# keychera/raytracing-clj

Hardware: AMD Instinct MI355X
Metric: Mray-samples/sec at 1200×675×100spp depth50; achieved HBM GB/s vs peak (higher is better)
Workload: dtype fp32

## Files before the change

raytracing-clj_amd/csrc/bvh.cpp:

```cpp
#include "bvh.h"

#include <algorithm>
#include <climits>
#include <cmath>
#include <numeric>

namespace rtclj {

float g_bvh_big_ratio = 4.0f;

namespace {

struct Box {
  float lo[3] = {INFINITY, INFINITY, INFINITY};
  float hi[3] = {-INFINITY, -INFINITY, -INFINITY};
  void add(const Box& b) {
    for (int k = 0; k < 3; ++k) {
      lo[k] = std::min(lo[k], b.lo[k]);
      hi[k] = std::max(hi[k], b.hi[k]);
    }
  }
};

Box body_box(const float* s) {
// ... 142 lines not shown
    std::nth_element(tmp.begin(), tmp.begin() + n / 2, tmp.end());
    med = tmp[n / 2];
  }
  Builder b{sph, {}, out};
  b.leaf_size = leaf_size;
  b.sah = sah;
  std::vector<char> is_big(n, 0);
  for (int i = 0; i < n; ++i) {
    const bool finite = std::isfinite(sph[4 * i]) && std::isfinite(sph[4 * i + 1]) &&
                        std::isfinite(sph[4 * i + 2]) && std::isfinite(sph[4 * i + 3]);
    if (!finite && out->big.size() < 64) {
      is_big[i] = 1;
      out->big.push_back(i);
    }
  }
  if (n > 8) {
    std::vector<int> order(n);
    std::iota(order.begin(), order.end(), 0);
    std::stable_sort(order.begin(), order.end(), [&](int x, int y) { return radii[x] > radii[y]; });
    int added = 0;
    for (int i : order) {
      if (added == kBvhBigMax || !(radii[i] > g_bvh_big_ratio * med)) break;
      if (is_big[i]) continue;
      is_big[i] = 1;
      out->big.push_back(i);
      ++added;
    }
  }
  std::sort(out->big.begin(), out->big.end());
  for (int i = 0; i < n; ++i)
    if (!is_big[i]) b.prim.push_back(i);
  Box all;
  for (int i : b.prim) all.add(body_box(sph + 4 * i));
  double bc[3] = {0, 0, 0}, br = 0;
  if (!b.prim.empty()) {
    for (int k = 0; k < 3; ++k) bc[k] = 0.5 * (double(all.lo[k]) + all.hi[k]);
    for (int i : b.prim) {
      const float* s = sph + 4 * i;
      const double dx = s[0] - bc[0], dy = s[1] - bc[1], dz = s[2] - bc[2];
      br = std::max(br, std::sqrt(dx * dx + dy * dy + dz * dz) + std::fabs(s[3]));
    }
  }
  for (int k = 0; k < 3; ++k) out->center[k] = static_cast<float>(bc[k]);
  out->radius = static_cast<float>(br * (1.0 + 1e-6)) + 1e-6f;
  out->nodes.emplace_back();
  const int cnt = static_cast<int>(b.prim.size());
  Box b0, b1;
  int c0 = 0, c1 = 0;
  if (cnt == 0) {
    c0 = c1 = b.leaf(0, 0, &b0);
    for (int k = 0; k < 3; ++k) b0.lo[k] = b0.hi[k] = 0.0f;
    b1 = b0;
  } else if (cnt <= leaf_size) {
    c0 = c1 = b.leaf(0, cnt, &b0);
    b1 = b0;
  } else {
    const int mid = b.split(0, cnt, 0);
    c0 = b.build(0, mid, 1, &b0);
    c1 = b.build(mid, cnt, 1, &b1);
  }
  BvhNode& root = out->nodes[0];
  set_box(root, 0, b0);
  set_box(root, 1, b1);
  root.child[0] = c0;
  root.child[1] = c1;
  for (BvhNode& nd : out->nodes) {
    float* ax[3] = {nd.x, nd.y, nd.z};
    for (int k = 0; k < 3; ++k)
      for (int c = 0; c < 2; ++c) {
        ax[k][c] = std::nextafter(static_cast<float>(double(ax[k][c]) - out->center[k]), -INFINITY);
        ax[k][2 + c] = std::nextafter(static_cast<float>(double(ax[k][2 + c]) - out->center[k]), INFINITY);
        ax[k][4 + c] = ax[k][c];
      }
  }
  out->depth = b.max_depth + 1;
  out->big_pair0 = static_cast<int>(out->pidx.size() / 2);
  const int nb = static_cast<int>(out->big.size());
// ... 11 lines not shown
```

raytracing-clj_amd/csrc/bvh.h:

```cpp
#pragma once
#include <cstdint>
#include <vector>

namespace rtclj {

struct alignas(16) BvhNode {
  float x[6], y[6], z[6];
  int child[2];
};
static_assert(sizeof(BvhNode) == 80, "BvhNode layout");

struct BvhHost {
  std::vector<BvhNode> nodes;
  std::vector<float> pairs;
  std::vector<int> pidx;
  std::vector<int> big;
  int big_pair0 = 0;
  int n_big_leaves = 0;
  float center[3] = {0, 0, 0};
  float radius = 0.0f;
  int depth = 0;
  int leaf_size = 2;
};

constexpr int kBvhStack = 16;
constexpr int kBvhBigMax = 8;

int bvh_build(const float* sphere, int n, BvhHost* out, int leaf_size = 2, bool sah = true);

}
```

raytracing-clj_amd/csrc/trace.hip:

```cpp
#include "trace_kernel.h"

#include <algorithm>
#include <chrono>
#include <atomic>
#include <climits>
#include <cstdlib>
#include <cmath>
#include <cstdint>
#include <cstring>
#include <mutex>
#include <string>
#include <thread>
#include <type_traits>
#include <vector>

namespace rtclj {

__device__ __forceinline__ int cost_bucket(unsigned c) {
  if (c < 8) return static_cast<int>(c);
  const int e = 31 - __clz(c);
  return ((e - 2) << 3) | static_cast<int>((c >> (e - 3)) & 7u);
}
__global__ __launch_bounds__(1024) void order_kernel(unsigned* __restrict__ cost, int* __restrict__ order,
                                                     int n) {
// ... 176 lines not shown
    case 28: return v28;
  }
#ifdef RTCLJ_DIAG
  if (const Variant* d = diag_variant(v)) return *d;
#endif
  return none;
}
static std::atomic<int> g_variant{0};
static std::atomic<int> g_schedule{0};
static const bool g_bvh_sah = [] {
  const char* e = std::getenv("RTCLJ_BVH");
  return !(e && std::strcmp(e, "median") == 0);
}();
#ifdef RTCLJ_DIAG
static const bool g_timeline = [] {
  const char* e = std::getenv("RTCLJ_TIMELINE");
  return e && std::atoi(e) != 0;
}();
#endif
constexpr int kDbg = 32;
constexpr int kDbgDevices = 64;
static std::mutex g_dbg_mu;
static unsigned long long* g_dbg[kDbgDevices] = {};
static unsigned long long* g_dbgw[kDbgDevices] = {};

}

using namespace rtclj;

struct DTree {
  float4* blob;
  int blob_f4, off_pairs, off_pidx, big_pair0, n_big_leaves, depth, n_nodes;
  float c[3], r;
};

struct ScheduleKey {
  int width, rows, row_begin, row_tile, tile_first, tile_step, gx, gy;
};
struct Schedule {
  hipStream_t stream = nullptr;
  unsigned* cost = nullptr;
  int* order = nullptr;
  int cap = 0;
  bool ready = false;
  bool sort_pending = false;
  int sort_plan = -1;
  ScheduleKey key{};
  unsigned long long* part = nullptr;
  size_t part_cap = 0;
  bool part_dirty = false;
  unsigned long long* word = nullptr;
  unsigned* done = nullptr;
  unsigned long long* sum = nullptr;
  int steal_cap = 0;
  int* owner = nullptr;
  int owner_cap = 0;
  unsigned long long* stealc = nullptr;
  unsigned epoch = 0;
  bool epoch_started = false;
  int2* units = nullptr;
  int units_cap = 0;
  int plan_units = -1;
  uint4* xq = nullptr;
  size_t xq_cap = 0;
  unsigned* xq_n = nullptr;
  unsigned long long xq_launches = 0;
// ... 171 lines not shown
    std::thread th[2];
    for (int k = 1; k < 3; ++k) th[k - 1] = std::thread([&, k] { bvh_build(s->sphere, n, &bvhs[k], 2 << k, g_bvh_sah); });
    bvh_build(s->sphere, n, &bvhs[0], 2, g_bvh_sah);
    for (std::thread& t : th) t.join();
  }
  hipError_t e = hipMalloc(&d->geo, n_pad * sizeof(float4));
  for (int k = 0; k < 3 && e == hipSuccess; ++k) {
    BvhHost& bvh = bvhs[k];
    const size_t nb = bvh.nodes.size() * sizeof(BvhNode);
    const size_t pb = bvh.pairs.size() * sizeof(float);
    const size_t isz = k == 2 ? sizeof(uint16_t) : sizeof(int);
    std::vector<uint16_t> pidx16(bvh.pidx.size());
    for (size_t i = 0; i < pidx16.size(); ++i) pidx16[i] = static_cast<uint16_t>(bvh.pidx[i]);
    const size_t ib = ((bvh.pidx.size() * isz + 15) / 16) * 16;
    std::vector<char> blob(nb + pb + ib, 0);
    if (k == 1)
      for (BvhNode& nd : bvh.nodes)
        for (int& c : nd.child)
          if (c >= 0) c *= static_cast<int>(sizeof(BvhNode));
    std::memcpy(blob.data(), bvh.nodes.data(), nb);
    std::memcpy(blob.data() + nb, bvh.pairs.data(), pb);
    if (k == 2) std::memcpy(blob.data() + nb + pb, pidx16.data(), pidx16.size() * sizeof(uint16_t));
    else std::memcpy(blob.data() + nb + pb, bvh.pidx.data(), bvh.pidx.size() * sizeof(int));
    DTree& t = d->tree[k];
    t.blob_f4 = static_cast<int>(blob.size() / 16);
    t.off_pairs = static_cast<int>(nb);
    t.off_pidx = static_cast<int>(nb + pb);
    t.big_pair0 = bvh.big_pair0;
    t.n_big_leaves = bvh.n_big_leaves;
    t.depth = bvh.depth;
    t.n_nodes = static_cast<int>(bvh.nodes.size());
    for (int j = 0; j < 3; ++j) t.c[j] = bvh.center[j];
    t.r = bvh.radius;
    e = hipMalloc(&t.blob, blob.size());
    if (e == hipSuccess) e = hipMemcpy(t.blob, blob.data(), blob.size(), hipMemcpyHostToDevice);
  }
  if (e == hipSuccess) e = hipMalloc(&d->geo2, n_pad * sizeof(float4));
  if (e == hipSuccess) e = hipMemcpy(d->geo2, geo2.data(), n_pad * sizeof(float4), hipMemcpyHostToDevice);
  if (e == hipSuccess) e = hipMalloc(&d->sph, cnt * sizeof(float4));
  if (e == hipSuccess) e = hipMalloc(&d->mat, cnt * sizeof(float4));
  if (e == hipSuccess) e = hipMalloc(&d->kind, cnt * sizeof(int));
  if (e == hipSuccess) e = hipMemcpy(d->geo, geo.data(), n_pad * sizeof(float4), hipMemcpyHostToDevice);
  if (e == hipSuccess) e = hipMemcpy(d->sph, sph.data(), cnt * sizeof(float4), hipMemcpyHostToDevice);
  if (e == hipSuccess) e = hipMemcpy(d->mat, mat.data(), cnt * sizeof(float4), hipMemcpyHostToDevice);
  if (e == hipSuccess) e = hipMemcpy(d->kind, kind.data(), cnt * sizeof(int), hipMemcpyHostToDevice);
  if (e != hipSuccess) {
    rt_scene_free(d);
    return hip_fail(e, "rt_scene_upload");
  }
  {
    std::lock_guard<std::mutex> lk(g_scenes_mu);
    g_scenes.push_back(d);
  }
  *out = d;
  return RT_OK;
}

extern "C" int rt_scene_free(rt_dscene* d) {
  if (!d) return RT_OK;
  {
    std::lock_guard<std::mutex> lk(g_scenes_mu);
    g_scenes.erase(std::remove(g_scenes.begin(), g_scenes.end(), d), g_scenes.end());
  }
  (void)hipSetDevice(d->device);
  if (d->geo) (void)hipFree(d->geo);
  if (d->geo2) (void)hipFree(d->geo2);
// ... 225 lines not shown
  std::memcpy(a.cam + 12, c->disk_u, 12);
  std::memcpy(a.cam + 15, c->disk_v, 12);
  a.defocus = c->defocus ? 1 : 0;
  a.n = ds->n;
  a.n_pad = ds->n_pad;
  a.width = p->width;
  a.rows_out = rows;
  a.row_begin = p->row_begin;
  a.row_tile = p->row_tile > 0 ? p->row_tile : 8;
  a.tile_first = p->tile_first;
  a.tile_step = p->tile_step;
  a.spp = p->spp;
  a.sample_begin = p->sample_begin;
  a.max_depth = p->max_depth;
  a.realm = (p->flags & RT_FLAG_REALM) ? 1 : 0;
  a.sampler = (p->flags & RT_FLAG_REJECTION_SAMPLERS) ? 0 : (RT_SAMPLER_SPHERE | RT_SAMPLER_DISK);
  a.key = seed_key(p->seed);
  if (rows == 0) return RT_OK;
  HIP_TRY(hipSetDevice(ds->device));
  int vsel = launch_variant(*ds, *p);
  if (variant_table(vsel).scan == SCAN_BVHS && p->max_depth > 1023) vsel = 16;
  const Variant& v = variant_table(vsel);
  if (!v.fn) return set_error(RT_E_ARG, "rt_launch: no kernel for variant " + std::to_string(vsel));
  const DTree& tr = ds->tree[variant_tree(vsel)];
  a.bvh_blob = tr.blob;
  a.bvh_blob_f4 = tr.blob_f4;
  a.bvh_off_pairs = tr.off_pairs;
  a.bvh_off_pidx = tr.off_pidx;
  a.big_pair0 = tr.big_pair0;
  a.n_big_leaves = tr.n_big_leaves;
  a.bvh_stack = compact_variant(vsel) ? stack_entries_compact(tr) : stack_entries(tr, variant_tree(vsel));
  for (int k = 0; k < 3; ++k) a.bvh_c[k] = tr.c[k];
  a.bvh_r = tr.r;
  {
    const int words = a.bvh_stack * 16 * (v.scan == SCAN_BVHO || v.scan == SCAN_BVHQ7 ? 1 : 2);
    a.mb_paths = std::min(32, words / kMbFields);
    a.compact = is_bvh_scan(v.scan) ? std::min(a.mb_paths, env_int("RTCLJ_COMPACT", a.mb_paths, 0)) : 0;
  }
  hipStream_t stream = static_cast<hipStream_t>(hip_stream);
  const int th = variant_rows(v);
  const int gx = (p->width + kTile - 1) / kTile, gy = (rows + th - 1) / th;
  const dim3 block(v.threads);
  const int n_tiles = gx * gy;
  a.tiles_x = gx;
  if (v.stats) {
    const int rc = dbg_buffers(ds->device, &a.dbg, &a.dbgw);
    if (rc != RT_OK) return rc;
  }
#ifdef RTCLJ_DIAG
  else if (g_timeline) {
    unsigned long long* unused = nullptr;
    const int rc = dbg_buffers(ds->device, &unused, &a.dbgw);
    if (rc != RT_OK) return rc;
  }
#endif
#ifdef RTCLJ_DIAG
  const size_t lds = launch_lds(*ds, vsel) + static_cast<size_t>(env_int("RTCLJ_LDS_PAD", 0, 0));
#else
  const size_t lds = launch_lds(*ds, vsel);
#endif
  if (lds > 64 * 1024) {
    HIP_TRY(hipFuncSetAttribute(v.fn, hipFuncAttributeMaxDynamicSharedMemorySize, static_cast<int>(lds)));
    if (v.sweep) HIP_TRY(hipFuncSetAttribute(v.sweep, hipFuncAttributeMaxDynamicSharedMemorySize, static_cast<int>(lds)));
  }
  Schedule* sch = nullptr;
  std::unique_lock<std::mutex> sched_lock;
// ... 344 lines not shown
```

raytracing-clj_amd/csrc/trace_diag.hip:

```cpp
#include "trace_kernel.h"

namespace rtclj {

template <int SRC, int SCAN, class F>
__device__ void diag_scan(const KArgs& a, const float4* s_geo, float ox, float oy, float oz, float ux, float uy,
                          float uz, F&& consider) {
  const int n = a.n;
  if constexpr (SCAN == SCAN_SIMPLE) {
#pragma unroll 1
    for (int s = 0; s < n; ++s) {
      float4 g;
      if constexpr (SRC == SRC_LDS) g = s_geo[s];
      else g = a.geo[s];
      const float ocx = g.x - ox, ocy = g.y - oy, ocz = g.z - oz;
      const float h = fmaf(uz, ocz, fmaf(uy, ocy, ux * ocx));
      const float c = fmaf(ocx, ocx, fmaf(ocz, ocz, fmaf(ocy, ocy, g.w)));
      const float disc = fmaf(h, h, -c);
      if ((disc >= 0.0f) & ((h >= 0.0f) | (c < 0.0f))) consider(h, disc, s);
    }
  } else {
    const Pair* tab;
    if constexpr (SRC == SRC_LDS) tab = reinterpret_cast<const Pair*>(s_geo);
    else tab = a.geo2;
    const f2 ox2 = {ox, ox}, oy2 = {oy, oy}, oz2 = {oz, oz};
// ... 231 lines not shown
        ox = cx;
        oy = cy;
        oz = cz;
      }
      dx = sx - ox;
      dy = sy - oy;
      dz = sz - oz;
      tr = tg = tb = 1.0f;
      rem = a.max_depth;
      last = -1;
      j = -1;
    }
    bool done = false;
    --rem;
    ++segs;
    const float len = sqrt_rn(fmaf(dz, dz, fmaf(dy, dy, dx * dx)));
    const float il = 1.0f / len;
    const float ux = dx * il, uy = dy * il, uz = dz * il;
    const float tmin = 1e-3f * len;
    float best_t = INFINITY;
    int best = -1;
    {
      auto consider_tie = [&](float h, float disc, int s) {
        const float sq = (s == last) ? fabsf(h) : sqrt_rn(disc);
        const float tn = h - sq;
        const float t = tn > tmin ? tn : h + sq;
        const uint64_t kk = (static_cast<uint64_t>(__float_as_uint(t)) << 32) | static_cast<uint32_t>(s);
        const uint64_t bkey = (static_cast<uint64_t>(__float_as_uint(best_t)) << 32) | static_cast<uint32_t>(best);
        const bool acc = (t > tmin) & (kk < bkey);
        best_t = acc ? t : best_t;
        best = acc ? s : best;
      };
      const float ecx = ox - a.bvh_c[0], ecy = oy - a.bvh_c[1], ecz = oz - a.bvh_c[2];
      const float D = __builtin_amdgcn_sqrtf(fmaf(ecz, ecz, fmaf(ecy, ecy, ecx * ecx))) + a.bvh_r;
      const float P = fmaf(2e-3f, D, 1e-6f);
      const float rux = __builtin_amdgcn_fmed3f(__builtin_amdgcn_rcpf(ux), -1e24f, 1e24f);
      const float ruy = __builtin_amdgcn_fmed3f(__builtin_amdgcn_rcpf(uy), -1e24f, 1e24f);
      const float ruz = __builtin_amdgcn_fmed3f(__builtin_amdgcn_rcpf(uz), -1e24f, 1e24f);
      f2 r_xy = {rux, ruy}, r_z = {ruz, ruz};
      const float nlx = -(ecx + P) * rux, nly = -(ecy + P) * ruy, nlz = -(ecz + P) * ruz;
      const float nhx = -(ecx - P) * rux, nhy = -(ecy - P) * ruy, nhz = -(ecz - P) * ruz;
      const bool sx = rux < 0.0f, sy = ruy < 0.0f, sz = ruz < 0.0f;
      f2 nf_x = {sx ? nhx : nlx, sx ? nlx : nhx};
      f2 nf_y = {sy ? nhy : nly, sy ? nly : nhy};
      f2 nf_z = {sz ? nhz : nlz, sz ? nlz : nhz};
      const int offx = sx ? 8 : 0, offy = 24 + (sy ? 8 : 0), offz = 48 + (sz ? 8 : 0);
      f2 o_xy = {ox, oy}, o_zux = {oz, ux}, u_yz = {uy, uz};
      auto leaf = [&](int p) {
        float hh[4], dd[4];
        int ii[4];
        unsigned nc[4];
        const Pair* const lp = pairs + p;
        const int2* const li = pidx + p;
#pragma unroll
        for (int qq = 0; qq < 2; ++qq) {
          const Pair g = lp[qq];
          const int2 id = li[qq];
          asm volatile("" : "+v"(o_xy), "+v"(o_zux), "+v"(u_yz));
          const f2 ocx = g.x - bc_lo(o_xy), ocy = g.y - bc_hi(o_xy), ocz = g.z - bc_lo(o_zux);
          const f2 h = fma2(bc_hi(u_yz), ocz, fma2(bc_lo(u_yz), ocy, bc_hi(o_zux) * ocx));
          const f2 c = fma2(ocx, ocx, fma2(ocz, ocz, fma2(ocy, ocy, g.w)));
          const f2 disc = fma2(h, h, -c);
          hh[2 * qq] = h.x;
          hh[2 * qq + 1] = h.y;
          dd[2 * qq] = disc.x;
          dd[2 * qq + 1] = disc.y;
          ii[2 * qq] = id.x;
          ii[2 * qq + 1] = id.y;
          const float d0 = disc.x, d1 = disc.y, h0 = h.x, h1 = h.y, c0 = c.x, c1 = c.y;
          nc[2 * qq] = __builtin_amdgcn_bitop3_b32(__float_as_uint(d0), __float_as_uint(h0), __float_as_uint(c0), 0x0b);
          nc[2 * qq + 1] = __builtin_amdgcn_bitop3_b32(__float_as_uint(d1), __float_as_uint(h1), __float_as_uint(c1), 0x0b);
        }
        const unsigned b01 = __builtin_amdgcn_perm(nc[1], nc[0], 0x0c0c0b09u);
        const unsigned b23 = __builtin_amdgcn_perm(nc[3], nc[2], 0x0b090c0cu);
        unsigned m = __builtin_amdgcn_bitop3_b32(b01, b23, 0x01010101u, 0xa8);
        while (m) {
          const unsigned k = __builtin_ctz(m);
          m &= m - 1;
          float h = hh[0], d = dd[0];
          int s = ii[0];
#pragma unroll
          for (int jj = 1; jj < 4; ++jj) {
            h = k == static_cast<unsigned>(8 * jj) ? hh[jj] : h;
            d = k == static_cast<unsigned>(8 * jj) ? dd[jj] : d;
            s = k == static_cast<unsigned>(8 * jj) ? ii[jj] : s;
          }
          consider_tie(h, d, s);
        }
      };
      auto node_test = [&](int node, float& tn0, float& tn1, bool& hit0, bool& hit1, int& c0, int& c1) {
        const char* nb = reinterpret_cast<const char*>(nodes) + static_cast<unsigned>(node);
        const f2* ax = reinterpret_cast<const f2*>(nb + offx);
        const f2* ay = reinterpret_cast<const f2*>(nb + offy);
        const f2* az = reinterpret_cast<const f2*>(nb + offz);
        const int2 ch = *reinterpret_cast<const int2*>(nb + 72);
        asm volatile("" : "+v"(r_xy), "+v"(r_z), "+v"(nf_x), "+v"(nf_y), "+v"(nf_z));
        const f2 tnx = fma2(ax[0], bc_lo(r_xy), bc_lo(nf_x)), tfx = fma2(ax[1], bc_lo(r_xy), bc_hi(nf_x));
        const f2 tny = fma2(ay[0], bc_hi(r_xy), bc_lo(nf_y)), tfy = fma2(ay[1], bc_hi(r_xy), bc_hi(nf_y));
        const f2 tnz = fma2(az[0], bc_lo(r_z), bc_lo(nf_z)), tfz = fma2(az[1], bc_lo(r_z), bc_hi(nf_z));
        tn0 = fmaxf(fmaxf(tnx.x, tny.x), tnz.x);
        tn1 = fmaxf(fmaxf(tnx.y, tny.y), tnz.y);
        const float tf0 = fminf(fminf(tfx.x, tfy.x), tfz.x);
        const float tf1 = fminf(fminf(tfx.y, tfy.y), tfz.y);
        float ntn0, ntn1;
        asm("v_max_f32 %0, %1, %2" : "=v"(ntn0) : "v"(tn0), "v"(tmin));
        asm("v_max_f32 %0, %1, %2" : "=v"(ntn1) : "v"(tn1), "v"(tmin));
        hit0 = ntn0 <= fminf(tf0, best_t);
        hit1 = ntn1 <= fminf(tf1, best_t);
        c0 = ch.x;
        c1 = ch.y;
      };
      for (int b = 0; b < a.n_big_leaves; ++b) leaf(a.big_pair0 + b * 2);
      int node = 0;
      unsigned short* top = stk0;
      bool go = true;
      while (go) {
        float tn0, tn1;
        bool hit0, hit1;
        int c0, c1;
        node_test(node, tn0, tn1, hit0, hit1, c0, c1);
        const bool l0 = hit0 && c0 < 0, l1 = hit1 && c1 < 0;
        if (l0 || l1) {
          leaf(l0 ? ~c0 : ~c1);
          if (l0 && l1) leaf(~c1);
        }
        const bool i0 = hit0 && !l0, i1 = hit1 && !l1;
        const bool sw = tn1 < tn0;
        int nxt = (i0 && (!i1 || !sw)) ? c0 : c1;
        *top = static_cast<unsigned short>(sw ? c0 : c1);
        top += (i0 && i1) ? 64 : 0;
        if (!(i0 || i1)) {
          go = top != stk0;
// ... 174 lines not shown
```

raytracing-clj_amd/csrc/trace_kernel.h:

```cpp
#pragma once
#include <hip/hip_runtime.h>

#include <algorithm>
#include <chrono>
#include <atomic>
#include <climits>
#include <cstdlib>
#include <cmath>
#include <cstdint>
#include <cstring>
#include <mutex>
#include <string>
#include <thread>
#include <type_traits>
#include <vector>

#include "bvh.h"
#include "fp_rn.h"
#include "rt_internal.h"

namespace rtclj {

struct alignas(16) KArgs {
  const float4* geo;
  const struct Pair* geo2;
  const float4* sph;
  const float4* mat;
  const int* kind;
  float* out;
  unsigned long long* counters;
  unsigned long long* dbg;
  unsigned long long* dbgw;
  float cam[18];
  int defocus;
  int n;
  int n_pad;
  int width;
  int rows_out;
  int row_begin, row_tile, tile_first, tile_step;
  const float4* bvh_blob;
  int bvh_blob_f4;
  int bvh_off_pairs;
  int bvh_off_pidx;
  int big_pair0;
  int n_big_leaves;
  int bvh_stack;
  float bvh_c[3], bvh_r;
  const int* tile_order;
  unsigned* tile_cost;
  unsigned long long* part;
  int tiles_x;
  int n_whole, split;
  const int2* unit_tab;
  uint64_t rt_magic;
  int spp, sample_begin, max_depth;
  int realm;
  int sampler;
  uint32_t key;
  unsigned long long* word;
  unsigned* done;
  unsigned long long* sum;
  int* owner;
  unsigned long long* stealc;
  int n_owner;
  int n_units;
  int share_from;
  int steal_min;
  int batch_max;
  int lds_batch_max;
  unsigned epoch;
  int compact;
  int mb_paths;
  uint4* xq;
  unsigned* xq_n;
};

__device__ __forceinline__ float rng_uniform(uint32_t& s) {
  s ^= s << 13;
  s ^= s >> 17;
  s ^= s << 5;
// ... 704 lines not shown
          ++st_blk;
          st_blk_lanes += __popcll(ex);
        }
      }
      const float sq = (s == last) ? fabsf(h) : sqrt_rn(disc);
      float t = h - sq;
      if (!(t > tmin)) t = h + sq;
      if (t > tmin && t < best_t) {
        best_t = t;
        best = s;
      }
    };
    if constexpr (SCAN == SCAN_SIMPLE || SCAN == SCAN_PK4) {
      diag_scan<SRC, SCAN>(a, s_geo, ox, oy, oz, ux, uy, uz, consider);
    } else if constexpr (is_bvh_scan(SCAN)) {
      auto consider_tie = [&](float h, float disc, int s) {
        if constexpr (STATS) st_fl += 3;
        if constexpr (STATS) ++st_blk_lanes;
        const float sq = (s == last) ? fabsf(h) : sqrt_rn(disc);
        const float tn = h - sq;
        const float t = tn > tmin ? tn : h + sq;
        const uint64_t key = (static_cast<uint64_t>(__float_as_uint(t)) << 32) | static_cast<uint32_t>(s);
        const uint64_t bkey = (static_cast<uint64_t>(__float_as_uint(best_t)) << 32) | static_cast<uint32_t>(best);
        const bool acc = (t > tmin) & (key < bkey);
        best_t = acc ? t : best_t;
        best = acc ? s : best;
      };
      const char* base = SRC == SRC_LDS ? reinterpret_cast<const char*>(s_geo)
                                        : reinterpret_cast<const char*>(a.bvh_blob);
      const KNode* nodes = reinterpret_cast<const KNode*>(base);
      const Pair* pairs = reinterpret_cast<const Pair*>(base + a.bvh_off_pairs);
      using PidxT = std::conditional_t<SCAN == SCAN_BVHO, ushort2, int2>;
      const PidxT* pidx = reinterpret_cast<const PidxT*>(base + a.bvh_off_pidx);
      const float ecx = ox - a.bvh_c[0], ecy = oy - a.bvh_c[1], ecz = oz - a.bvh_c[2];
      const float D = __builtin_amdgcn_sqrtf(fmaf(ecz, ecz, fmaf(ecy, ecy, ecx * ecx))) + a.bvh_r;
      const float P = fmaf(2e-3f, D, 1e-6f);
      if constexpr (STATS) st_fl += 27;
      const float rux = __builtin_amdgcn_fmed3f(__builtin_amdgcn_rcpf(ux), -1e24f, 1e24f);
      const float ruy = __builtin_amdgcn_fmed3f(__builtin_amdgcn_rcpf(uy), -1e24f, 1e24f);
      const float ruz = __builtin_amdgcn_fmed3f(__builtin_amdgcn_rcpf(uz), -1e24f, 1e24f);
      f2 r_xy = {rux, ruy}, r_z = {ruz, ruz};
      const float nlx = -(ecx + P) * rux, nly = -(ecy + P) * ruy, nlz = -(ecz + P) * ruz;
      const float nhx = -(ecx - P) * rux, nhy = -(ecy - P) * ruy, nhz = -(ecz - P) * ruz;
      const bool sx = rux < 0.0f, sy = ruy < 0.0f, sz = ruz < 0.0f;
      f2 nf_x = {sx ? nhx : nlx, sx ? nlx : nhx};
      f2 nf_y = {sy ? nhy : nly, sy ? nly : nhy};
      f2 nf_z = {sz ? nhz : nlz, sz ? nlz : nhz};
      const int offx = sx ? 8 : 0, offy = 24 + (sy ? 8 : 0), offz = 48 + (sz ? 8 : 0);
      f2 o_xy = {ox, oy}, o_zux = {oz, ux}, u_yz = {uy, uz};
      constexpr bool kLeafRec = SRC == SRC_LDS && is_q(SCAN);
      auto leaf = [&](int p) {
        RT_MARK("leaf");
        if constexpr (STATS) {
          ++st_blk;
          const uint64_t ex = __builtin_amdgcn_read_exec();
          if (lane == __ffsll(static_cast<long long>(ex)) - 1) ++st_leafw;
        }
        constexpr int NPL = leaf_pairs(SCAN);
        constexpr int NP = NPL > 2 ? 2 : NPL;
        if constexpr (kLeafRec) {
          unsigned pa = static_cast<unsigned>(p);
          asm volatile("" : "+v"(pa));
          auto body = [&](unsigned addr, float& h, float& c, float& disc) {
            const f4v g = *(LdsF4)(uintptr_t)addr;
            const float ocx = g.x - o_xy.x, ocy = g.y - o_xy.y, ocz = g.z - o_zux.x;
            h = fmaf(u_yz.y, ocz, fmaf(u_yz.x, ocy, o_zux.y * ocx));
            c = fmaf(ocx, ocx, fmaf(ocz, ocz, fmaf(ocy, ocy, g.w)));
            disc = fmaf(h, h, -c);
          };
          asm volatile("" : "+v"(o_xy), "+v"(o_zux), "+v"(u_yz));
          unsigned nc[4];
#pragma unroll
          for (int j = 0; j < 4; ++j) {
            if constexpr (STATS) st_fl += 16;
            float h, c, disc;
            body(pa + 16u * j, h, c, disc);
            nc[j] = __builtin_amdgcn_bitop3_b32(__float_as_uint(disc), __float_as_uint(h), __float_as_uint(c), 0x0b);
          }
          const unsigned b01 = __builtin_amdgcn_perm(nc[1], nc[0], 0x0c0c0b09u);
          const unsigned b23 = __builtin_amdgcn_perm(nc[3], nc[2], 0x0b090c0cu);
          unsigned m = __builtin_amdgcn_bitop3_b32(b01, b23, 0x01010101u, 0xa8);
// ... 65 lines not shown
          float h = hh[0], d = dd[0];
          int s = ii[0];
#pragma unroll
          for (int j = 1; j < 2 * NP; ++j) {
            h = k == static_cast<unsigned>(8 * j) ? hh[j] : h;
            d = k == static_cast<unsigned>(8 * j) ? dd[j] : d;
            s = k == static_cast<unsigned>(8 * j) ? ii[j] : s;
          }
          consider_tie(h, d, s);
        }
        }
      };
      auto node_planes = [&](int node, float& tn0, float& tn1, float& tf0, float& tf1, int& c0, int& c1) {
        if constexpr (STATS) st_fl += 24;
        const unsigned nof = SCAN == SCAN_BVHQ    ? static_cast<unsigned>(node)
                             : SCAN == SCAN_BVHQ7 ? __umul24(static_cast<unsigned>(node), 80u) + lds_addr(nodes)
                                                  : __umul24(static_cast<unsigned>(node), 80u);
        f2 x0, x1, y0, y1, z0, z1;
        int2 ch;
        if constexpr (SRC == SRC_LDS && is_q(SCAN)) {
          const LdsF2 lx = (LdsF2)(uintptr_t)(nof + offx), ly = (LdsF2)(uintptr_t)(nof + offy),
                      lz = (LdsF2)(uintptr_t)(nof + offz);
          x0 = lx[0], x1 = lx[1], y0 = ly[0], y1 = ly[1], z0 = lz[0], z1 = lz[1];
          const long long c2 = *(LdsI64)(uintptr_t)(nof + 72);
          ch = make_int2(static_cast<int>(c2), static_cast<int>(c2 >> 32));
        } else {
          const char* nb = reinterpret_cast<const char*>(nodes) + nof;
          const f2* ax = reinterpret_cast<const f2*>(nb + offx);
          const f2* ay = reinterpret_cast<const f2*>(nb + offy);
          const f2* az = reinterpret_cast<const f2*>(nb + offz);
          x0 = ax[0], x1 = ax[1], y0 = ay[0], y1 = ay[1], z0 = az[0], z1 = az[1];
          ch = *reinterpret_cast<const int2*>(nb + 72);
        }
        asm volatile("" : "+v"(r_xy), "+v"(r_z), "+v"(nf_x), "+v"(nf_y), "+v"(nf_z));
        f2 tnx, tfx, tny, tfy, tnz, tfz;
#pragma unroll
        for (int e = 0; e < 2; ++e) {
          tnx[e] = fma3(x0[e], r_xy.x, nf_x.x);
          tfx[e] = fma3(x1[e], r_xy.x, nf_x.y);
          tny[e] = fma3(y0[e], r_xy.y, nf_y.x);
          tfy[e] = fma3(y1[e], r_xy.y, nf_y.y);
          tnz[e] = fma3(z0[e], r_z.x, nf_z.x);
          tfz[e] = fma3(z1[e], r_z.x, nf_z.y);
        }
        tn0 = fmaxf(fmaxf(tnx.x, tny.x), tnz.x);
        tn1 = fmaxf(fmaxf(tnx.y, tny.y), tnz.y);
        tf0 = fminf(fminf(tfx.x, tfy.x), tfz.x);
        tf1 = fminf(fminf(tfx.y, tfy.y), tfz.y);
        c0 = ch.x;
        c1 = ch.y;
      };
      auto node_test = [&](int node, float& tn0, float& tn1, bool& hit0, bool& hit1, int& c0, int& c1) {
        float tf0, tf1;
        node_planes(node, tn0, tn1, tf0, tf1, c0, c1);
        float tb0, tb1;
        asm("v_min_f32 %0, %1, %2" : "=v"(tb0) : "v"(tf0), "v"(best_t));
        asm("v_min_f32 %0, %1, %2" : "=v"(tb1) : "v"(tf1), "v"(best_t));
        hit0 = !(tn0 > tb0) & !(tmin > tf0);
        hit1 = !(tn1 > tb1) & !(tmin > tf1);
      };
      RT_MARK("bigleaf");
      for (int b = 0; b < a.n_big_leaves; ++b) {
        if constexpr (kLeafRec)
          leaf(static_cast<int>(lds_addr(nodes)) + a.bvh_off_pairs + ((a.big_pair0 >> 1) + b) * kLeafRecBytes);
        else
          leaf(a.big_pair0 + b * leaf_pairs(SCAN));
      }
      RT_MARK("tree_setup");
      int node = SRC == SRC_LDS && SCAN == SCAN_BVHQ ? static_cast<int>(lds_addr(nodes)) : 0;
      StackT* const stk0 = s_stack + threadIdx.x;
      StackT* top = stk0;
      int row_b = NT * static_cast<int>(sizeof(StackT));
      asm volatile("" : "+v"(row_b));
      bool go = true;
      while (go) {
        RT_MARK("node");
        if constexpr (STATS) {
          ++st_sph;
          const uint64_t ex = __builtin_amdgcn_read_exec();
          if (lane == __ffsll(static_cast<long long>(ex)) - 1) {
            ++st_trav;
            st_trav_lanes += __popcll(ex);
          }
        }
        float tn0, tn1;
        bool hit0, hit1;
        int c0, c1;
        node_test(node, tn0, tn1, hit0, hit1, c0, c1);
        const bool l0 = hit0 && c0 < 0, l1 = hit1 && c1 < 0;
        if (l0 || l1) {
          leaf(l0 ? ~c0 : ~c1);
          if (l0 && l1) leaf(~c1);
        }
        const bool i0 = hit0 && !l0, i1 = hit1 && !l1;
        const bool sw = tn1 < tn0;
        int nxt = (i0 && (!i1 || !sw)) ? c0 : c1;
        *top = static_cast<StackT>(sw ? c0 : c1);
        top = reinterpret_cast<StackT*>(reinterpret_cast<char*>(top) + ((i0 && i1) ? row_b : 0));
        if (!(i0 || i1)) {
          top -= NT;
          go = top >= stk0;
          nxt = *top;
        }
        node = nxt;
      }
      RT_MARK("hit");
      ox = o_xy.x;
      oy = o_xy.y;
      oz = o_zux.x;
      ux = o_zux.y;
      uy = u_yz.x;
      uz = u_yz.y;
    } else {
      auto load = [&](int s) -> float4 {
        if constexpr (SRC == SRC_LDS) return s_geo[s];
        else return a.geo[s];
      };
      float4 g0 = load(0), g1 = load(1), g2 = load(2), g3 = load(3);
      for (int s = 0; s < n; s += 4) {
        const float4 n0 = load(s + 4), n1 = load(s + 5), n2 = load(s + 6), n3 = load(s + 7);
        float h[4], disc[4];
        bool cand[4];
#pragma unroll
        for (int k = 0; k < 4; ++k) {
          const float4 g = k == 0 ? g0 : k == 1 ? g1 : k == 2 ? g2 : g3;
          const float ocx = g.x - ox, ocy = g.y - oy, ocz = g.z - oz;
          h[k] = fmaf(uz, ocz, fmaf(uy, ocy, ux * ocx));
          const float c = fmaf(ocx, ocx, fmaf(ocz, ocz, fmaf(ocy, ocy, g.w)));
          disc[k] = fmaf(h[k], h[k], -c);
          cand[k] = fminf(disc[k], fmaxf(h[k], -c)) >= 0.0f;
        }
        if (cand[0] | cand[1] | cand[2] | cand[3]) {
#pragma unroll
          for (int k = 0; k < 4; ++k)
// ... 418 lines not shown
```

Measured before the change: 17250.

## Replace slab-test padding with per-axis reciprocal padding and drop stack base register

Reworks the ray-box slab test setup: instead of a fixed padding P scaled by distance, the ray now computes a padding that may be derived from the maximum body radius and applies separate near/far reciprocals per axis with a direction-dependent bias. The BVH builder records the largest primitive radius to feed this bound. Node-test arithmetic is restructured into helper functions, and the stack termination check compares against the shared stack base instead of a per-thread base pointer, freeing a register. This aims to tighten or stabilise traversal bounds and reduce register pressure, at the cost of slightly more per-ray setup and a changed conservativeness of the box test.

```diff
diff --git a/raytracing-clj_amd/csrc/bvh.cpp b/raytracing-clj_amd/csrc/bvh.cpp
--- a/raytracing-clj_amd/csrc/bvh.cpp
+++ b/raytracing-clj_amd/csrc/bvh.cpp
@@ -198,17 +198,19 @@
     if (!is_big[i]) b.prim.push_back(i);
   Box all;
   for (int i : b.prim) all.add(body_box(sph + 4 * i));
-  double bc[3] = {0, 0, 0}, br = 0;
+  double bc[3] = {0, 0, 0}, br = 0, rmax = 0;
   if (!b.prim.empty()) {
     for (int k = 0; k < 3; ++k) bc[k] = 0.5 * (double(all.lo[k]) + all.hi[k]);
     for (int i : b.prim) {
       const float* s = sph + 4 * i;
       const double dx = s[0] - bc[0], dy = s[1] - bc[1], dz = s[2] - bc[2];
       br = std::max(br, std::sqrt(dx * dx + dy * dy + dz * dz) + std::fabs(s[3]));
+      rmax = std::max(rmax, double(std::fabs(s[3])));
     }
   }
   for (int k = 0; k < 3; ++k) out->center[k] = static_cast<float>(bc[k]);
   out->radius = static_cast<float>(br * (1.0 + 1e-6)) + 1e-6f;
+  out->r_max = static_cast<float>(rmax * (1.0 + 1e-6));
   out->nodes.emplace_back();
   const int cnt = static_cast<int>(b.prim.size());
   Box b0, b1;
diff --git a/raytracing-clj_amd/csrc/bvh.h b/raytracing-clj_amd/csrc/bvh.h
--- a/raytracing-clj_amd/csrc/bvh.h
+++ b/raytracing-clj_amd/csrc/bvh.h
@@ -19,6 +19,7 @@
   int n_big_leaves = 0;
   float center[3] = {0, 0, 0};
   float radius = 0.0f;
+  float r_max = 0.0f;
   int depth = 0;
   int leaf_size = 2;
 };
diff --git a/raytracing-clj_amd/csrc/bvh_pad.h b/raytracing-clj_amd/csrc/bvh_pad.h
--- /dev/null
+++ b/raytracing-clj_amd/csrc/bvh_pad.h
@@ -0,0 +1,140 @@
+#pragma once
+#include <cmath>
+
+#if defined(__HIPCC__)
+#define RT_PAD_FN __host__ __device__ __forceinline__
+#else
+#define RT_PAD_FN inline
+#endif
+
+namespace rtclj {
+
+constexpr float kPadK = 2e-3f;
+constexpr float kPadLimit = 3e-3f;
+constexpr float kPadRound = 2e-3f;
+constexpr float kPadRmax = 3.0f;
+constexpr float kPadAbs = 5e-4f;
+
+RT_PAD_FN float pad_rcp(float x) {
+#if defined(__HIP_DEVICE_COMPILE__)
+  return __builtin_amdgcn_rcpf(x);
+#else
+  return 1.0f / x;
+#endif
+}
+RT_PAD_FN float pad_sqrt(float x) {
+#if defined(__HIP_DEVICE_COMPILE__)
+  return __builtin_amdgcn_sqrtf(x);
+#else
+  return std::sqrt(x);
+#endif
+}
+RT_PAD_FN unsigned pad_u(float x) { return __builtin_bit_cast(unsigned, x); }
+RT_PAD_FN float pad_f(unsigned x) { return __builtin_bit_cast(float, x); }
+RT_PAD_FN unsigned pad_sel(unsigned m, unsigned a, unsigned b) {
+#if defined(__HIP_DEVICE_COMPILE__)
+  return __builtin_amdgcn_bitop3_b32(a, b, m, 0xe4);
+#else
+  return (a & m) | (b & ~m);
+#endif
+}
+RT_PAD_FN float pad_fma(float a, float b, float c) {
+#if defined(__HIP_DEVICE_COMPILE__)
+  float r;
+  asm("v_fma_f32 %0, %1, %2, %3" : "=v"(r) : "v"(a), "v"(b), "v"(c));
+  return r;
+#else
+  return std::fma(a, b, c);
+#endif
+}
+
+template <unsigned L>
+RT_PAD_FN unsigned pad_and(unsigned x) {
+#if defined(__HIP_DEVICE_COMPILE__)
+  unsigned r;
+  asm("v_and_b32 %0, %1, %2" : "=v"(r) : "n"(L), "v"(x));
+  return r;
+#else
+  return x & L;
+#endif
+}
+template <unsigned L>
+RT_PAD_FN unsigned pad_or(unsigned x) {
+#if defined(__HIP_DEVICE_COMPILE__)
+  unsigned r;
+  asm("v_or_b32 %0, %1, %2" : "=v"(r) : "n"(L), "v"(x));
+  return r;
+#else
+  return x | L;
+#endif
+}
+template <unsigned L>
+RT_PAD_FN unsigned pad_rsub(unsigned x) {
+#if defined(__HIP_DEVICE_COMPILE__)
+  unsigned r;
+  asm("v_sub_u32 %0, %1, %2" : "=v"(r) : "n"(L), "v"(x));
+  return r;
+#else
+  return L - x;
+#endif
+}
+RT_PAD_FN unsigned pad_neg_mask(unsigned x) { return static_cast<unsigned>(static_cast<int>(x) >> 31); }
+
+
+struct PadRay {
+  float p;
+  unsigned kn, kf;
+  unsigned per_t;
+};
+RT_PAD_FN PadRay pad_ray(float ex, float ey, float ez, float ux, float uy, float uz, float R, float c0_bodies,
+                         bool allow_per_t = true) {
+  constexpr unsigned kLimBits = __builtin_bit_cast(unsigned, kPadLimit), kKBits = __builtin_bit_cast(unsigned, kPadK),
+                     kTinyBits = __builtin_bit_cast(unsigned, 1e-24f);
+  const float D = pad_sqrt(fmaf(ez, ez, fmaf(ey, ey, ex * ex))) + R + kPadAbs;
+  const float P = kPadK * D;
+  const float pc = kPadK * fmaf(kPadRound, D, c0_bodies);
+  PadRay r;
+  const float umin = fminf(fminf(fabsf(ux), fabsf(uy)), fabsf(uz));
+  r.per_t = allow_per_t ? pad_neg_mask(pad_u(pc) - pad_u(P)) & pad_neg_mask(pad_rsub<kLimBits>(pad_u(umin))) : 0u;
+  r.p = pad_f(pad_sel(r.per_t, pad_u(pc), pad_u(P)));
+  r.kn = kTinyBits + (pad_and<kKBits - kTinyBits>(r.per_t));
+  r.kf = r.kn ^ pad_and<0x80000000u>(r.per_t);
+  return r;
+}
+
+struct PadAxis {
+  float mn, mf, on, of;
+  unsigned sign;
+};
+RT_PAD_FN PadAxis pad_axis(float u, float e, float tmin, const PadRay& r) {
+  PadAxis a;
+  a.sign = pad_and<0x80000000u>(pad_u(u));
+  const unsigned skn = a.sign | r.kn;
+  a.mn = pad_rcp(u + pad_f(skn));
+  a.mf = pad_rcp(u + pad_f(a.sign ^ r.kf));
+  const float sp = pad_f(a.sign | pad_u(r.p));
+  a.on = -(e + sp) * a.mn;
+  a.of = fmaf(-(e - sp), a.mf, tmin);
+  return a;
+}
+
+RT_PAD_FN void pad_interval(const PadAxis& x, const PadAxis& y, const PadAxis& z, float xn, float xf, float yn,
+                            float yf, float zn, float zf, float& tn, float& tf) {
+  const float tnx = pad_fma(xn, x.mn, x.on), tfx = pad_fma(xf, x.mf, x.of);
+  const float tny = pad_fma(yn, y.mn, y.on), tfy = pad_fma(yf, y.mf, y.of);
+  const float tnz = pad_fma(zn, z.mn, z.on), tfz = pad_fma(zf, z.mf, z.of);
+  tn = fmaxf(fmaxf(tnx, tny), tnz);
+  tf = fminf(fminf(tfx, tfy), tfz);
+}
+
+RT_PAD_FN bool pad_meets(float tn, float tf, float tmin, float best_t) {
+  float tb;
+#if defined(__HIP_DEVICE_COMPILE__)
+  asm("v_min_f32 %0, %1, %2" : "=v"(tb) : "v"(tf), "v"(best_t));
+#else
+  tb = tf < best_t ? tf : best_t;
+#endif
+  return !(tn > tb) & !(tmin > tf);
+}
+
+}
diff --git a/raytracing-clj_amd/csrc/trace.hip b/raytracing-clj_amd/csrc/trace.hip
--- a/raytracing-clj_amd/csrc/trace.hip
+++ b/raytracing-clj_amd/csrc/trace.hip
@@ -232,6 +232,7 @@
   float4* blob;
   int blob_f4, off_pairs, off_pidx, big_pair0, n_big_leaves, depth, n_nodes;
   float c[3], r;
+  float c0;
 };
 
 struct ScheduleKey {
@@ -469,6 +470,7 @@
     t.n_nodes = static_cast<int>(bvh.nodes.size());
     for (int j = 0; j < 3; ++j) t.c[j] = bvh.center[j];
     t.r = bvh.radius;
+    t.c0 = kPadRmax * bvh.r_max;
     e = hipMalloc(&t.blob, blob.size());
     if (e == hipSuccess) e = hipMemcpy(t.blob, blob.data(), blob.size(), hipMemcpyHostToDevice);
   }
@@ -760,6 +762,7 @@
   a.bvh_stack = compact_variant(vsel) ? stack_entries_compact(tr) : stack_entries(tr, variant_tree(vsel));
   for (int k = 0; k < 3; ++k) a.bvh_c[k] = tr.c[k];
   a.bvh_r = tr.r;
+  a.bvh_c0 = tr.c0;
   {
     const int words = a.bvh_stack * 16 * (v.scan == SCAN_BVHO || v.scan == SCAN_BVHQ7 ? 1 : 2);
     a.mb_paths = std::min(32, words / kMbFields);
diff --git a/raytracing-clj_amd/csrc/trace_diag.hip b/raytracing-clj_amd/csrc/trace_diag.hip
--- a/raytracing-clj_amd/csrc/trace_diag.hip
+++ b/raytracing-clj_amd/csrc/trace_diag.hip
@@ -287,19 +287,12 @@
         best = acc ? s : best;
       };
       const float ecx = ox - a.bvh_c[0], ecy = oy - a.bvh_c[1], ecz = oz - a.bvh_c[2];
-      const float D = __builtin_amdgcn_sqrtf(fmaf(ecz, ecz, fmaf(ecy, ecy, ecx * ecx))) + a.bvh_r;
-      const float P = fmaf(2e-3f, D, 1e-6f);
-      const float rux = __builtin_amdgcn_fmed3f(__builtin_amdgcn_rcpf(ux), -1e24f, 1e24f);
-      const float ruy = __builtin_amdgcn_fmed3f(__builtin_amdgcn_rcpf(uy), -1e24f, 1e24f);
-      const float ruz = __builtin_amdgcn_fmed3f(__builtin_amdgcn_rcpf(uz), -1e24f, 1e24f);
-      f2 r_xy = {rux, ruy}, r_z = {ruz, ruz};
-      const float nlx = -(ecx + P) * rux, nly = -(ecy + P) * ruy, nlz = -(ecz + P) * ruz;
-      const float nhx = -(ecx - P) * rux, nhy = -(ecy - P) * ruy, nhz = -(ecz - P) * ruz;
-      const bool sx = rux < 0.0f, sy = ruy < 0.0f, sz = ruz < 0.0f;
-      f2 nf_x = {sx ? nhx : nlx, sx ? nlx : nhx};
-      f2 nf_y = {sy ? nhy : nly, sy ? nly : nhy};
-      f2 nf_z = {sz ? nhz : nlz, sz ? nlz : nhz};
-      const int offx = sx ? 8 : 0, offy = 24 + (sy ? 8 : 0), offz = 48 + (sz ? 8 : 0);
+      const PadRay pr = pad_ray(ecx, ecy, ecz, ux, uy, uz, a.bvh_r, a.bvh_c0);
+      const PadAxis pax = pad_axis(ux, ecx, tmin, pr), pay = pad_axis(uy, ecy, tmin, pr), paz = pad_axis(uz, ecz, tmin, pr);
+      f2 r_x = {pax.mn, pax.mf}, r_y = {pay.mn, pay.mf}, r_z = {paz.mn, paz.mf};
+      f2 nf_x = {pax.on, pax.of}, nf_y = {pay.on, pay.of}, nf_z = {paz.on, paz.of};
+      const int offx = static_cast<int>(pax.sign >> 28), offy = 24 + static_cast<int>(pay.sign >> 28),
+                offz = 48 + static_cast<int>(paz.sign >> 28);
       f2 o_xy = {ox, oy}, o_zux = {oz, ux}, u_yz = {uy, uz};
       auto leaf = [&](int p) {
         float hh[4], dd[4];
@@ -349,10 +342,10 @@
         const f2* ay = reinterpret_cast<const f2*>(nb + offy);
         const f2* az = reinterpret_cast<const f2*>(nb + offz);
         const int2 ch = *reinterpret_cast<const int2*>(nb + 72);
-        asm volatile("" : "+v"(r_xy), "+v"(r_z), "+v"(nf_x), "+v"(nf_y), "+v"(nf_z));
-        const f2 tnx = fma2(ax[0], bc_lo(r_xy), bc_lo(nf_x)), tfx = fma2(ax[1], bc_lo(r_xy), bc_hi(nf_x));
-        const f2 tny = fma2(ay[0], bc_hi(r_xy), bc_lo(nf_y)), tfy = fma2(ay[1], bc_hi(r_xy), bc_hi(nf_y));
-        const f2 tnz = fma2(az[0], bc_lo(r_z), bc_lo(nf_z)), tfz = fma2(az[1], bc_lo(r_z), bc_hi(nf_z));
+        asm volatile("" : "+v"(r_x), "+v"(r_y), "+v"(r_z), "+v"(nf_x), "+v"(nf_y), "+v"(nf_z));
+        const f2 tnx = fma2(ax[0], bc_lo(r_x), bc_lo(nf_x)), tfx = fma2(ax[1], bc_hi(r_x), bc_hi(nf_x));
+        const f2 tny = fma2(ay[0], bc_lo(r_y), bc_lo(nf_y)), tfy = fma2(ay[1], bc_hi(r_y), bc_hi(nf_y));
+        const f2 tnz = fma2(az[0], bc_lo(r_z), bc_lo(nf_z)), tfz = fma2(az[1], bc_hi(r_z), bc_hi(nf_z));
         tn0 = fmaxf(fmaxf(tnx.x, tny.x), tnz.x);
         tn1 = fmaxf(fmaxf(tnx.y, tny.y), tnz.y);
         const float tf0 = fminf(fminf(tfx.x, tfy.x), tfz.x);
diff --git a/raytracing-clj_amd/csrc/trace_kernel.h b/raytracing-clj_amd/csrc/trace_kernel.h
--- a/raytracing-clj_amd/csrc/trace_kernel.h
+++ b/raytracing-clj_amd/csrc/trace_kernel.h
@@ -16,6 +16,7 @@
 #include <vector>
 
 #include "bvh.h"
+#include "bvh_pad.h"
 #include "fp_rn.h"
 #include "rt_internal.h"
 
@@ -46,6 +47,7 @@
   int n_big_leaves;
   int bvh_stack;
   float bvh_c[3], bvh_r;
+  float bvh_c0;
   const int* tile_order;
   unsigned* tile_cost;
   unsigned long long* part;
@@ -816,21 +818,15 @@
       const Pair* pairs = reinterpret_cast<const Pair*>(base + a.bvh_off_pairs);
       using PidxT = std::conditional_t<SCAN == SCAN_BVHO, ushort2, int2>;
       const PidxT* pidx = reinterpret_cast<const PidxT*>(base + a.bvh_off_pidx);
+      constexpr bool kPadPerT = true;
       const float ecx = ox - a.bvh_c[0], ecy = oy - a.bvh_c[1], ecz = oz - a.bvh_c[2];
-      const float D = __builtin_amdgcn_sqrtf(fmaf(ecz, ecz, fmaf(ecy, ecy, ecx * ecx))) + a.bvh_r;
-      const float P = fmaf(2e-3f, D, 1e-6f);
-      if constexpr (STATS) st_fl += 27;
-      const float rux = __builtin_amdgcn_fmed3f(__builtin_amdgcn_rcpf(ux), -1e24f, 1e24f);
-      const float ruy = __builtin_amdgcn_fmed3f(__builtin_amdgcn_rcpf(uy), -1e24f, 1e24f);
-      const float ruz = __builtin_amdgcn_fmed3f(__builtin_amdgcn_rcpf(uz), -1e24f, 1e24f);
-      f2 r_xy = {rux, ruy}, r_z = {ruz, ruz};
-      const float nlx = -(ecx + P) * rux, nly = -(ecy + P) * ruy, nlz = -(ecz + P) * ruz;
-      const float nhx = -(ecx - P) * rux, nhy = -(ecy - P) * ruy, nhz = -(ecz - P) * ruz;
-      const bool sx = rux < 0.0f, sy = ruy < 0.0f, sz = ruz < 0.0f;
-      f2 nf_x = {sx ? nhx : nlx, sx ? nlx : nhx};
-      f2 nf_y = {sy ? nhy : nly, sy ? nly : nhy};
-      f2 nf_z = {sz ? nhz : nlz, sz ? nlz : nhz};
-      const int offx = sx ? 8 : 0, offy = 24 + (sy ? 8 : 0), offz = 48 + (sz ? 8 : 0);
+      const PadRay pr = pad_ray(ecx, ecy, ecz, ux, uy, uz, a.bvh_r, a.bvh_c0, kPadPerT);
+      if constexpr (STATS) st_fl += 36;
+      const PadAxis pax = pad_axis(ux, ecx, tmin, pr), pay = pad_axis(uy, ecy, tmin, pr), paz = pad_axis(uz, ecz, tmin, pr);
+      f2 r_x = {pax.mn, pax.mf}, r_y = {pay.mn, pay.mf}, r_z = {paz.mn, paz.mf};
+      f2 nf_x = {pax.on, pax.of}, nf_y = {pay.on, pay.of}, nf_z = {paz.on, paz.of};
+      const int offx = static_cast<int>(pax.sign >> 28), offy = 24 + static_cast<int>(pay.sign >> 28),
+                offz = 48 + static_cast<int>(paz.sign >> 28);
       f2 o_xy = {ox, oy}, o_zux = {oz, ux}, u_yz = {uy, uz};
       constexpr bool kLeafRec = SRC == SRC_LDS && is_q(SCAN);
       auto leaf = [&](int p) {
@@ -962,32 +958,19 @@
           x0 = ax[0], x1 = ax[1], y0 = ay[0], y1 = ay[1], z0 = az[0], z1 = az[1];
           ch = *reinterpret_cast<const int2*>(nb + 72);
         }
-        asm volatile("" : "+v"(r_xy), "+v"(r_z), "+v"(nf_x), "+v"(nf_y), "+v"(nf_z));
-        f2 tnx, tfx, tny, tfy, tnz, tfz;
-#pragma unroll
-        for (int e = 0; e < 2; ++e) {
-          tnx[e] = fma3(x0[e], r_xy.x, nf_x.x);
-          tfx[e] = fma3(x1[e], r_xy.x, nf_x.y);
-          tny[e] = fma3(y0[e], r_xy.y, nf_y.x);
-          tfy[e] = fma3(y1[e], r_xy.y, nf_y.y);
-          tnz[e] = fma3(z0[e], r_z.x, nf_z.x);
-          tfz[e] = fma3(z1[e], r_z.x, nf_z.y);
-        }
-        tn0 = fmaxf(fmaxf(tnx.x, tny.x), tnz.x);
-        tn1 = fmaxf(fmaxf(tnx.y, tny.y), tnz.y);
-        tf0 = fminf(fminf(tfx.x, tfy.x), tfz.x);
-        tf1 = fminf(fminf(tfx.y, tfy.y), tfz.y);
+        asm volatile("" : "+v"(r_x), "+v"(r_y), "+v"(r_z), "+v"(nf_x), "+v"(nf_y), "+v"(nf_z));
+        const PadAxis px = {r_x.x, r_x.y, nf_x.x, nf_x.y, 0}, py = {r_y.x, r_y.y, nf_y.x, nf_y.y, 0},
+                      pz = {r_z.x, r_z.y, nf_z.x, nf_z.y, 0};
+        pad_interval(px, py, pz, x0.x, x1.x, y0.x, y1.x, z0.x, z1.x, tn0, tf0);
+        pad_interval(px, py, pz, x0.y, x1.y, y0.y, y1.y, z0.y, z1.y, tn1, tf1);
         c0 = ch.x;
         c1 = ch.y;
       };
       auto node_test = [&](int node, float& tn0, float& tn1, bool& hit0, bool& hit1, int& c0, int& c1) {
         float tf0, tf1;
         node_planes(node, tn0, tn1, tf0, tf1, c0, c1);
-        float tb0, tb1;
-        asm("v_min_f32 %0, %1, %2" : "=v"(tb0) : "v"(tf0), "v"(best_t));
-        asm("v_min_f32 %0, %1, %2" : "=v"(tb1) : "v"(tf1), "v"(best_t));
-        hit0 = !(tn0 > tb0) & !(tmin > tf0);
-        hit1 = !(tn1 > tb1) & !(tmin > tf1);
+        hit0 = pad_meets(tn0, tf0, tmin, best_t);
+        hit1 = pad_meets(tn1, tf1, tmin, best_t);
       };
       RT_MARK("bigleaf");
       for (int b = 0; b < a.n_big_leaves; ++b) {
@@ -998,8 +981,9 @@
       }
       RT_MARK("tree_setup");
       int node = SRC == SRC_LDS && SCAN == SCAN_BVHQ ? static_cast<int>(lds_addr(nodes)) : 0;
-      StackT* const stk0 = s_stack + threadIdx.x;
-      StackT* top = stk0;
+      unsigned tix = threadIdx.x;
+      asm volatile("" : "+v"(tix));
+      StackT* top = s_stack + tix;
       int row_b = NT * static_cast<int>(sizeof(StackT));
       asm volatile("" : "+v"(row_b));
       bool go = true;
@@ -1029,7 +1013,7 @@
         top = reinterpret_cast<StackT*>(reinterpret_cast<char*>(top) + ((i0 && i1) ? row_b : 0));
         if (!(i0 || i1)) {
           top -= NT;
-          go = top >= stk0;
+          go = top >= s_stack;
           nxt = *top;
         }
         node = nxt;
```

New measurement: 17540 (median of 6 runs). 1.02x the previous value.
